# cgmb/euler

Hardware: AMD Instinct MI355X
Metric: cells*steps/sec of sim_step() (frames incl. the PCG pressure projection) + pressure-solve HBM GB/s vs roofline (higher is better)
Workload: dtype f64

## Files before the change

euler_amd/csrc/k_pcg.h:

```cpp
#pragma once

#include "euler_dev.h"
#include "k_mg.h"

#define COMM_CALL(expr) do { if ((expr) != 0) { eu_set_error("communicator callback failed: %s", #expr); return EULER_ECOMM; } } while (0)
#define LOC(ptr) ((ptr) + S->e_lo)
enum { SW_FACTOR = 0, SW_FORWARD = 1, SW_BACKWARD = 2 };

int eu_launch_build_system(euler_sim* S, float dt);
int eu_launch_velocity_update(euler_sim* S, float dt, int finish);
int eu_launch_band_ranges(euler_sim* S);
int eu_launch_sweep(euler_sim* S, int op, int cls, int force, int fin_qq = -1);
int eu_launch_factor_tile(euler_sim* S, int force);
int eu_launch_precond_tile(euler_sim* S, int rupd, int sweeps, int fin_dot, int force, double alpha, bool r_only = false, int zform = -1);
int eu_launch_search_apply(euler_sim* S, int it);
int eu_launch_finish_p(euler_sim* S);
int eu_launch_dot(euler_sim* S, const double* a, const double* b, int fin_op, int force);
int eu_comm_exchange(euler_sim* S, double* send_lo, double* send_hi, double* recv_lo, double* recv_hi, int count, double* small, int nsmall);
int eu_comm_finish(euler_sim* S, int fin_op, int is_max, int force);
int eu_comm_halo_two(euler_sim* S, double* a, double* b);
bool tile_recompute(const euler_sim* S);
int p_steps(const euler_sim* S);

enum { FIN_SIGMA_INIT = 0, FIN_ALPHA, FIN_RNORM, FIN_BETA, FIN_STORE_ONLY, FIN_TO_COMM };
#define FIN_VIA_P2P 0x100

static inline bool tile_fused(const euler_sim* S) { return eu_is_tile(S) && S->cfg.sweep_mode != EULER_SWEEP_SIMPLE; }
static inline bool ghost_mode(const euler_sim* S) { return S->has_comm && !S->p2p_on && tile_fused(S); }
enum { XR_ZSEND_LO = 0, XR_ZSEND_HI, XR_ZRECV_LO, XR_ZRECV_HI, XR_GS_LO0, XR_GS_LO1, XR_GS_HI0, XR_GS_HI1 };
static inline double* xrow(const euler_sim* S, int k) { return S->xrows + (size_t)k * S->xrow_len; }
static inline int sa_run(const euler_sim* S) {
  if (S->opt[EULER_OPT_SA_RUN] != 8 && !S->has_comm && !eu_is_two_level(S)) return (int)S->opt[EULER_OPT_SA_RUN];
  return 8;
}
static inline bool tile_z_recompute(const euler_sim* S) {
  return tile_recompute(S) && tile_fused(S) && !eu_is_two_level(S) && S->tile_w == 16 && !S->has_comm && !S->slab_on && S->band_lo == 0 &&
         S->opt[EULER_OPT_TILE_STORE_Z] == 0 && S->chunk_list && S->tile_table;
}
static inline int fin_or_comm(const euler_sim* S, int fin_op) {
  return S->has_comm ? (S->p2p_on ? (fin_op | FIN_VIA_P2P) : (int)FIN_TO_COMM) : fin_op;
}

#ifdef __HIPCC__
#define RED_THREADS 1024
typedef double sw_d2 __attribute__((ext_vector_type(2)));

__device__ __forceinline__ bool pcg_idle(const PcgScalars* sc) { return sc->done || !sc->nonzero; }

#define DPP_WAVE_SHL1 0x130
#define DPP_WAVE_SHR1 0x138

template <int CTRL>
__device__ __forceinline__ double wave_shift_inject(double v, double edge) {
  const int lo = __builtin_amdgcn_update_dpp(__double2loint(edge), __double2loint(v), CTRL, 0xf, 0xf, false);
  const int hi = __builtin_amdgcn_update_dpp(__double2hiint(edge), __double2hiint(v), CTRL, 0xf, 0xf, false);
  return __hiloint2double(hi, lo);
}


__device__ __forceinline__ void pcg_scalar_step(PcgScalars* sc, int op, double v) {
  switch (op) {
    case FIN_SIGMA_INIT: sc->sigma = v; break;
    case FIN_ALPHA: sc->zs = v; sc->alpha_prev = sc->alpha; sc->alpha = sc->sigma / v; sc->alpha_hist[sc->iters & 7] = sc->alpha; sc->iters += 1; break;
    case FIN_RNORM: sc->rnorm = v; if (v <= sc->tol) sc->done = 1; break;
    case FIN_BETA: sc->sigma_new = v; sc->beta = v / sc->sigma; sc->sigma = v; break;
    case FIN_TO_COMM: sc->comm_val = v; if (sc->comm_slot) *sc->comm_slot = v; break;
    default: sc->sigma_new = v; break;
// ... 113 lines not shown
  double* pre;
  const double* in;
  double* out;
  unsigned long long* granules;
  int gran_stride;
  const unsigned long long* xg_in;
  unsigned long long* xg_out;
  const int4* ranges;
  int band_lo, nb_local;
  int couple;
  unsigned int* ticket;
  unsigned int ticket_base;
  unsigned int epoch;
  const PcgScalars* sc;
  int force;
  int* error;
  unsigned long long* timeline;
  int tile_w;
  int fin_qq;
  double* qq_partial;
  unsigned int* qq_counter;
  PcgScalars* sc_w;
};

struct TileArgs {
  SkewGeom g;
  const uint8_t* mask;
  double* pre;
  double* r;
  const double* as;
  double* z;
  int band_lo, nb_local;
  int rupd;
  int sweeps;
  int fin_dot;
  int via;
  double* part_max; double* part_dot;
  unsigned int* counter;
  const unsigned int* list;
  const double* table;
  PcgScalars* sc;
  int force;
  double alpha_arg;
  double* pair_slot;
  double *zsend_lo, *zsend_hi;
  int edge_lo, edge_hi;
  int reverse;
  double* cpart;
  int cshift;
  int cmode, cnx, cny;
  const double *gs_lo, *gs_hi;
  int zform;
  double *zhalo, *zrows;
};

__device__ __forceinline__ double factor_step(double aa, double own, double nbv) {
  const double cl = -1.0 * own, cb = -1.0 * nbv;
  double e = aa - cl * cl - cb * cb;
  if (e < 0.25 * aa) e = (aa != 0.0) ? aa : 1.0;
  return 1.0 / sqrt(e);
}

template <int CTRL>
__device__ __forceinline__ double dpp_move(double v) {
  const int lo = __builtin_amdgcn_update_dpp(0, __double2loint(v), CTRL, 0xf, 0xf, true);
  const int hi = __builtin_amdgcn_update_dpp(0, __double2hiint(v), CTRL, 0xf, 0xf, true);
  return __hiloint2double(hi, lo);
}
__device__ __forceinline__ double group_sum(double v) {
  v = v + dpp_move<0xB1>(v);
  v = v + dpp_move<0x4E>(v);
  if (MG_LG == 8) v = v + dpp_move<0x141>(v);
  return v;
}
#endif
```

euler_amd/csrc/k_pcg.hip:

```cpp
#include "k_pcg.h"

#include <cmath>
#include <vector>

template <bool IS_MAX>
__global__ __launch_bounds__(RED_THREADS) void k_reduce_final(const double* __restrict__ partial, int n, PcgScalars* sc,
                                                              int op, int force) {
  if (!force && pcg_idle(sc)) return;
  double v = 0.0;
  for (int i = threadIdx.x; i < n; i += RED_THREADS) {
    const double w = partial[i];
    if (IS_MAX) v = w > v ? w : v; else v += w;
  }
  v = IS_MAX ? block_max(v) : block_sum(v);
  if (threadIdx.x == 0) pcg_scalar_step(sc, op, v);
}

template <bool EDGES>
__global__ __launch_bounds__(RED_THREADS) void k_dot_partial(const double* __restrict__ a, const double* __restrict__ b,
                                                             const uint8_t* __restrict__ mask, size_t S,
                                                             double* __restrict__ partial, PcgScalars* sc, int force,
                                                             unsigned int* counter, int fin_op, int TS, int nb_local, int edges) {
  if (!force && pcg_idle(sc)) return;
  const size_t chunk = (((S + gridDim.x - 1) / gridDim.x) + 1) & ~(size_t)1;
// ... 471 lines not shown
    hipLaunchKernelGGL(k_nonzero_to_comm, dim3(1), dim3(1), 0, S->stream, S->sc);
    COMM_CALL(S->comm.allreduce(S->comm.ctx, &S->sc->comm_val, 1, 1));
    hipLaunchKernelGGL(k_nonzero_from_comm, dim3(1), dim3(1), 0, S->stream, S->sc);
  }
  return EULER_OK;
}

static int project_resident(euler_sim* S, float dt, Solve& v) {
  const bool res_skip = S->res_skip_once != 0;
  S->res_skip_once = 0;
  if (!res_skip && eu_resident_eligible(S)) {
    const unsigned int cap_chunks = 4u * (unsigned int)eu_resident_capacity(S, S->cfg.pcg_precision == EULER_PCG_F32);
    unsigned int guess = S->res_last_chunks;
    if (!S->res_have_last) {
      HIPCHK(hipMemcpyAsync(S->sc_host, S->sc, sizeof(PcgScalars), hipMemcpyDeviceToHost, S->stream));
      HIPCHK(hipStreamSynchronize(S->stream));
      guess = S->sc_host->n_chunks;
    }
    if (guess + guess / 16 + 8 <= cap_chunks || S->cfg.pcg_precision == EULER_PCG_F32) {
      v.solved = true;
      S->prof_iter = -2;
      if (int rc = eu_launch_resident(S, cap_chunks)) return rc;
      HIPCHK(hipMemcpyAsync(S->sc_host, S->sc, sizeof(PcgScalars), hipMemcpyDeviceToHost, S->stream));
      HIPCHK(hipStreamSynchronize(S->stream));
      S->res_last_chunks = S->sc_host->n_chunks; S->res_have_last = 1;
      const int err = *S->res_err;
      if (err == 0) {
        if (S->sc_host->nonzero) { S->res_solves += 1; S->pcg_fields_resident = 1; }
        return eu_launch_velocity_update(S, dt, 0);
      }
      *S->res_err = 0;
      if (S->cfg.pcg_precision == EULER_PCG_F32 && err == 2) { eu_set_error("EULER_PCG_F32: the solve's active chunks do not fit the resident solver"); return EULER_EHIP; }
      if (err != 2) { S->res_fallbacks += 1; S->res_disabled = 1; }
      S->solve_seq -= 1;
      S->lean_ok = 0;
      S->res_skip_once = 1;
      *S->sc_host = v.prev;
      return eu_launch_project(S, dt);
    }
  }
  return EULER_OK;
}

static int project_first_direction(euler_sim* S, Solve& v) {
  int rc;
  const bool tile = tile_fused(S), two_level = tile && eu_is_two_level(S);
  if (two_level && S->has_comm && !(eu_is_mg(S) && ghost_mode(S) && S->slab_on)) {
    eu_set_error("coarse-correction preconditioners with several ranks: EULER_PRECOND_IC0_TILE_MG on row slabs without mailboxes only");
    return EULER_EINVAL;
  }
  if (two_level && (rc = eu_launch_coarse_setup(S))) return rc;
  if (two_level && (rc = eu_launch_coarse_consistent(S))) return rc;
  v.zr = tile && tile_z_begin(S);
  if (tile) {
    if ((rc = eu_launch_factor_tile(S, 0))) return rc;
    if ((rc = eu_launch_precond_tile(S, 0, 1, FIN_SIGMA_INIT, 0, 0.0))) return rc;
  } else {
  if (S->cfg.precond != EULER_PRECOND_JACOBI && (rc = eu_launch_sweep(S, SW_FACTOR, KC_PRECON_FACTOR, 0))) return rc;
  if ((rc = launch_precondition(S, 0, FIN_SIGMA_INIT))) return rc;
  }
  if ((rc = ring_begin(S))) return rc;
  if (first_direction_folded(S)) {
    const PcgScalars& ps = v.prev;
    if (ps.nonzero && !(std::isfinite(ps.alpha) && std::isfinite(ps.beta) && std::isfinite(ps.rnorm) && std::isfinite(ps.sigma) && std::isfinite(ps.zs)))
      for (int k = 0; k < S->s_ring_n; ++k) HIPCHK(hipMemsetAsync(S->s_ring[k] + S->skew_off, 0, S->Sw * sizeof(double), S->stream));
  }
  else if (two_level) { if ((rc = eu_launch_coarse_search_init(S))) return rc; }
  else
  LAUNCH(S, KC_UPDATE_SEARCH, k_update_search<true>, dim3(eu_blocks(S->e_cnt, 256 * 4, 4096)), dim3(256), LOC(S->s), LOC(S->z),
         LOC(S->cellmask), S->e_cnt, S->sc, 0, 0.0);
  if (S->has_comm && eu_p2p_has_neighbour_arrays(S)) {
    const int y0 = S->band_lo > 0 ? 64 * S->band_lo : -1, y1 = S->band_hi < S->geom.nbands ? 64 * S->band_hi - 1 : -1;
    LAUNCH(S, KC_UPDATE_SEARCH, k_publish_edge_rows, dim3((S->X + 255) / 256, 2), dim3(256), S->s, S->geom, y0, y1, S->sc);
  }
  if (S->s_ring_n == 2) HIPCHK(hipMemsetAsync(LOC(S->s2), 0, S->e_cnt * sizeof(double), S->stream));
  S->s_stale = 1;
  return EULER_OK;
}

static int project_iterate(euler_sim* S, Solve& v) {
  int rc;
  HIPCHK(hipMemcpyAsync(S->sc_host, S->sc, sizeof(PcgScalars), hipMemcpyDeviceToHost, S->stream));
  HIPCHK(hipStreamSynchronize(S->stream));
  const int poll = S->cfg.pcg_poll_interval > 0 ? S->cfg.pcg_poll_interval : 8;
  const int max_it = S->cfg.max_iterations;
  const bool tile = tile_fused(S), fold0 = first_direction_folded(S);
  int it = 0, chunk = 0;
  bool stop = !S->sc_host->nonzero;
  S->s_none = stop ? 1 : 0;
  while (it < max_it && !stop) {
    int chunk_end = it + poll;
    if (!v.drain_poll && v.pred_iters > 0 && it < v.pred_iters + poll && chunk_end > v.pred_iters - 2) {
      const int lo = v.pred_iters - 2 < chunk_end ? v.pred_iters - 2 : chunk_end;
      chunk_end = lo > it + 2 ? lo : it + 2;
    }
    if (chunk_end > max_it) chunk_end = max_it;
    for (; it < chunk_end; ++it) {
      S->prof_iter = it;
      const bool fused = it > 0 || fold0;
      if (it == 0 && fold0) { S->s = S->s_ring[S->s_ring_n - 1]; S->s2 = S->s_ring[0]; }
      if ((rc = fused ? eu_launch_search_apply(S, it) : launch_apply_a_and_alpha(S, 0))) return rc;
      if (tile) {
        S->prof_iter = it;
        const int nx = it + 1, steps = S->s_ring_n;
        const bool next_odd = !(nx >= steps && nx % steps == 0);
        const int zform = v.zr && it + 1 < max_it ? (it + 2 < max_it && next_odd ? 1 : 0) : -1;
        if ((rc = eu_launch_precond_tile(S, 1, it + 1 < max_it, FIN_BETA, 0, 0.0, false, zform))) return rc;
        S->z_halo_last = zform == 1;
        v.zr_ran = v.zr_ran || zform == 1;
        continue;
      }
      S->tile_as_override = fused ? S->q : S->z;
      rc = eu_launch_precond_tile(S, 1, 0, -1, 0, 0.0, true);
      S->tile_as_override = nullptr;
      if (rc) return rc;
      if (it + 1 < max_it) {
        S->prof_iter = it + 1;
        if ((rc = launch_precondition(S, 0, FIN_BETA))) return rc;
      }
    }
    if (it < max_it && v.drain_poll) {
      HIPCHK(hipMemcpyAsync(S->sc_host, S->sc, sizeof(PcgScalars), hipMemcpyDeviceToHost, S->stream));
      HIPCHK(hipStreamSynchronize(S->stream));
      stop = S->sc_host->done != 0;
    } else
    if (it < max_it) {
      const int slot = chunk & 1;
      if (chunk > 0) {
        HIPCHK(hipEventSynchronize(S->poll_event[slot ^ 1]));
        stop = S->poll_host[slot ^ 1].done != 0;
      }
      HIPCHK(hipMemcpyAsync(&S->poll_host[slot], S->sc, sizeof(PcgScalars), hipMemcpyDeviceToHost, S->stream));
      HIPCHK(hipEventRecord(S->poll_event[slot], S->stream));
      ++chunk;
    }
  }
  return EULER_OK;
}

static int project_finish(euler_sim* S, float dt, const Solve& v) {
  int rc;
  S->prof_iter = -2;
  S->z_halo_last = 0;
  if (v.zr_ran && (rc = eu_launch_precond_tile(S, 0, 1, -1, 0, 0.0, false, 2))) return rc;
  const bool finish_in_update = !S->has_comm && !S->slab_on && S->opt[EULER_OPT_VELOCITY_TWO_PASS] == 0;
  if (!finish_in_update) { if ((rc = eu_launch_finish_p(S))) return rc; }
  if (S->s_ring_n > 2) { S->s = S->s_base[0]; S->s2 = S->s_base[1]; }
  if (S->has_comm && S->slab_on) {
    const int X = S->X, nbk = (X + 255) / 256;
    double *send_lo = S->halo_buf, *send_hi = S->halo_buf + X, *recv_lo = S->halo_buf + 2 * X, *recv_hi = S->halo_buf + 3 * X;
    if (S->band_lo > 0) hipLaunchKernelGGL(k_pack_row, dim3(nbk), dim3(256), 0, S->stream, S->p, send_lo, S->geom, S->band_lo, 0);
    COMM_CALL(S->bulk.halo(S->bulk.ctx, send_lo, send_hi, recv_lo, recv_hi, X));
    if (S->band_hi < S->geom.nbands) hipLaunchKernelGGL(k_unpack_row, dim3(nbk), dim3(256), 0, S->stream, S->p, recv_hi, S->geom, S->band_hi, 0);
  } else if (S->has_comm) {
    const int n = S->comm.nranks, nb = S->geom.nbands;
    std::vector<int64_t> off(n), cnt(n);
    for (int k = 0; k < n; ++k) {
      const int64_t lo = (int64_t)nb * k / n, hi = (int64_t)nb * (k + 1) / n;
      off[k] = lo * S->geom.TS * 64 * 8;
// ... 65 lines not shown
```

euler_amd/csrc/k_search.hip:

```cpp
#include "k_pcg.h"

#include <type_traits>

#define SA_THREADS 256
struct SaPair { sw_d2 z, so; double ez0, es0, ez1, es1; };

__device__ __forceinline__ double pick3(int t, int tb1, int tb2, double v0, double v1, double v2) {
  double v = v0;
  v = t >= tb1 ? v1 : v;
  v = t >= tb2 ? v2 : v;
  return v;
}
template <int SLAB, int PMODE, int SA_RUN, int COARSE = 0, bool STORE = true, bool ZR = false>
__global__ __launch_bounds__(SA_THREADS, (COARSE == 2 && PMODE == 1 && SLAB == 0) ? 4 : 1) void k_search_apply(const double* __restrict__ s_old, const double* __restrict__ z,
                                                             double* __restrict__ s_new, double* __restrict__ out,
                                                             const uint8_t* __restrict__ mask, SkewGeom g,
                                                             double* __restrict__ partial, PcgScalars* sc, int force,
                                                             unsigned int* counter, int fin_op, SlabNeighbours nbr,
                                                             double* __restrict__ p, double* s_new_base, double* s_old_base,
                                                             const unsigned int* __restrict__ chunk_list,
                                                             CoarseRef cref, SaHist hist, ZrArgs zr) {
  static_assert(PMODE == 1 || PMODE == 2 || PMODE == 4 || PMODE == 8, "PMODE: p is left alone (1) or takes the N fmadds that are due (the ring's length)");
  static_assert(!ZR || (SLAB == 0 && SA_RUN == 8 && COARSE == 0), "ZR: one GPU, runs of one tile, no coarse part");
  __shared__ double s_cy[COARSE == 2 ? SA_THREADS / 64 : 1][COARSE == 2 ? MG_NI + 1 : 1][64];
  __shared__ double s_ce[COARSE == 2 ? SA_THREADS / 64 : 1][COARSE == 2 ? MG_NI + 1 : 1][64];
  if (!force && pcg_idle(sc)) return;
  __shared__ sw_d2 s_ztab[ZR ? 8 : 1][64];
  if (ZR) {
    for (int k = threadIdx.x; k < 8 * 64; k += SA_THREADS) (&s_ztab[0][0])[k] = reinterpret_cast<const sw_d2*>(zr.table)[k];
    __syncthreads();
  }
  const double beta = sc->beta;
  (void)s_new_base; (void)s_old_base;
  constexpr int NPA = PMODE >= 2 ? PMODE : 2;
  double al[NPA] = {};
  if (PMODE >= 2) {
    const int k = sc->iters;
#pragma unroll
    for (int j = 0; j < NPA; ++j) al[j] = sc->alpha_hist[(k - NPA + j) & 7];
  }
  const int lane = threadIdx.x & 63;
  const int TS = g.TS, npairs = TS / 2;
  const int nb_local = (int)(g.S / ((size_t)TS * 64));
  const int cpb = (npairs + SA_RUN - 1) / SA_RUN, total = nb_local * cpb;
  const int n_waves = gridDim.x * (SA_THREADS / 64);
  const bool edge_lane = lane == 0 || lane == 63;
  double t = 0.0;
  const bool listed = chunk_list != nullptr;
  const int ntb16 = g.T / 16;
  const int todo = listed ? (int)sc->n_chunks : total;
  typedef std::integral_constant<bool, true> yes_t;
  typedef std::integral_constant<bool, false> no_t;
  for (int i = blockIdx.x * (SA_THREADS / 64) + (threadIdx.x >> 6); i < todo; i += n_waves) {
    int c = i, per = cpb;
    bool interior = false;
    if (listed) { const unsigned int ent = chunk_list[i]; interior = (ent & EU_CHUNK_INTERIOR) != 0; c = (int)(ent & ~EU_CHUNK_INTERIOR); per = ntb16; }
    const int lb = c / per, P0 = (c % per) * SA_RUN, P1 = ZR ? P0 + SA_RUN : (P0 + SA_RUN < npairs ? P0 + SA_RUN : npairs);
    const size_t bbase = (size_t)lb * TS * 64 + 2 * lane;
    auto run = [&](auto full_tag) {
      constexpr bool FULL = decltype(full_tag)::value;
      unsigned int mm[SA_RUN];
      unsigned int any = 0;
#pragma unroll
      for (int j = 0; j < SA_RUN; ++j) {
        if (FULL) mm[j] = CM_INTERIOR | (CM_INTERIOR << 8);
        else mm[j] = P0 + j < P1 ? (unsigned int)*reinterpret_cast<const unsigned short*>(mask + bbase + (size_t)(P0 + j) * 128) : 0u;
        any |= mm[j];
      }
      if (!FULL && !listed && !__ballot(((any | (any >> 8)) & CM_FLUID) != 0)) return;
      sw_d2 zz[ZR ? SA_RUN : 1];
      if (ZR) {
        sw_d2 rr[SA_RUN], pp[SA_RUN];
#pragma unroll
        for (int j = 0; j < SA_RUN; ++j) {
          rr[j] = *reinterpret_cast<const sw_d2*>(zr.r + bbase + (size_t)(P0 + j) * 128);
          pp[j] = FULL ? s_ztab[j][lane] : *reinterpret_cast<const sw_d2*>(zr.pre + bbase + (size_t)(P0 + j) * 128);
        }
        double none = 0.0;
        tile_solve<2 * SA_RUN, false>(mm, rr, pp, zz, none);
      }
      const int ztile = P0 / SA_RUN;
      const bool up_remote = SLAB == 1 && nbr.z_up && lb + 1 == nb_local, dn_remote = SLAB == 1 && nbr.z_dn && lb == 0;
      const double* ez = lane == 0 ? (dn_remote ? nbr.z_dn : z) : (up_remote ? nbr.z_up : z);
      const double* es = lane == 0 ? (dn_remote ? nbr.s_dn : s_old) : (up_remote ? nbr.s_up : s_old);
      const bool remote = lane == 0 ? dn_remote : up_remote;
      const long long e0_base = lane == 0 ? ((long long)(lb - 1) * TS + 62) * 64 + 127 : ((long long)(lb + 1) * TS - 64) * 64 + 1;
      const long long e1_base = lane == 0 ? ((long long)(lb - 1) * TS + 64) * 64 + 126 : ((long long)(lb + 1) * TS - 62) * 64;
      const unsigned int vbit = lane == 0 ? CM_DOWN : CM_UP;
      const bool ghost = SLAB == 2 && (lane == 0 ? (nbr.zrow_dn != nullptr && lb == 0) : (nbr.zrow_up != nullptr && lb + 1 == nb_local));
      const double* gz = lane == 0 ? nbr.zrow_dn : nbr.zrow_up;
      const double* gs = lane == 0 ? nbr.srow_dn : nbr.srow_up;
      double* gsn = lane == 0 ? nbr.snew_dn : nbr.snew_up;
      const int gcol = lane == 0 ? 0 : -63;
      const double* zrow = ZR ? zr.rows + (long long)(lane == 0 ? 2 * lb - 1 : 2 * lb + 2) * zr.X : nullptr;
      double cy0 = 0.0, cy1 = 0.0, cy2 = 0.0, ce0 = 0.0, ce1 = 0.0, ce2 = 0.0;
      double (*cyv)[64] = s_cy[COARSE == 2 ? threadIdx.x >> 6 : 0];
      double (*cev)[64] = s_ce[COARSE == 2 ? threadIdx.x >> 6 : 0];
      int ctb1 = 0x7fffffff, ctb2 = 0x7fffffff, cJb = 0;
      (void)cJb;
      if (COARSE == 2) {
        cJb = (2 * (P0 - 1) - lane - MG_G0 / 2) >> MG_LOG;
        ctb1 = MG_G0 * (cJb + 1) + lane + MG_G0 / 2;
        const int row = (cref.band0 + lb) * 64 + lane;
        const int hi_ = cref.nx - 1;
        int i0, i1;
        double fy;
        mg_cell_w(row, cref.ny, i0, i1, fy);
        const double* y0 = cref.y + (size_t)i0 * cref.nx;
        const double* y1 = cref.y + (size_t)i1 * cref.nx;
#pragma unroll
        for (int q = 0; q <= MG_NI; ++q) { const int c = cJb + q < 0 ? 0 : (cJb + q < hi_ ? cJb + q : hi_); cyv[q][lane] = mg_rows(y0[c], y1[c], fy); }
#pragma unroll
        for (int q = 0; q <= MG_NI; ++q) cev[q][lane] = 0.0;
        if (edge_lane) {
          const int re = row + (lane == 0 ? -1 : 1);
          if (re >= 0 && re < MG_G0 * cref.ny) {
            mg_cell_w(re, cref.ny, i0, i1, fy);
            y0 = cref.y + (size_t)i0 * cref.nx; y1 = cref.y + (size_t)i1 * cref.nx;
#pragma unroll
            for (int q = 0; q <= MG_NI; ++q) { const int c = cJb + q < 0 ? 0 : (cJb + q < hi_ ? cJb + q : hi_); cev[q][lane] = mg_rows(y0[c], y1[c], fy); }
          }
        }
// ... 40 lines not shown
            if (ZR) { d.ez0 = zrow[2 * P + gcol]; d.es0 = s_old[k]; }
            else if (SLAB == 2 && ghost) { d.ez0 = gz[2 * P + gcol]; d.es0 = gs[2 * P + gcol]; }
            else if (SLAB == 1 && remote) { d.ez0 = ld_system(ez + k); d.es0 = ld_system(es + k); } else { d.ez0 = ez[k]; d.es0 = es[k]; }
          }
          if (((m >> 8) & CM_FLUID) && ((m >> 8) & vbit)) {
            const long long k = e1_base + (long long)P * 128;
            if (ZR) { d.ez1 = zrow[2 * P + 1 + gcol]; d.es1 = s_old[k]; }
            else if (SLAB == 2 && ghost) { d.ez1 = gz[2 * P + 1 + gcol]; d.es1 = gs[2 * P + 1 + gcol]; }
            else if (SLAB == 1 && remote) { d.ez1 = ld_system(ez + k); d.es1 = ld_system(es + k); } else { d.ez1 = ez[k]; d.es1 = es[k]; }
          }
          if (COARSE == 1) {
            d.ez0 = d.ez0 + pick3(2 * P, ctb1, ctb2, ce0, ce1, ce2);
            d.ez1 = d.ez1 + pick3(2 * P + 1, ctb1, ctb2, ce0, ce1, ce2);
          }
          if (COARSE == 2) {
            d.ez0 = d.ez0 + p0y(2 * P, cev);
            d.ez1 = d.ez1 + p0y(2 * P + 1, cev);
          }
        }
        if (COARSE == 1) {
          d.z.x = d.z.x + pick3(2 * P, ctb1, ctb2, cy0, cy1, cy2);
          d.z.y = d.z.y + pick3(2 * P + 1, ctb1, ctb2, cy0, cy1, cy2);
        }
        if (COARSE == 2) {
          d.z.x = d.z.x + p0y(2 * P, cyv);
          d.z.y = d.z.y + p0y(2 * P + 1, cyv);
        }
      };
      auto sprime = [&](const SaPair& d) __attribute__((always_inline)) { return sw_d2{d.z.x + beta * d.so.x, d.z.y + beta * d.so.y}; };
      SaPair A, B, Cn;
      load_pair(P0 - 1, A, 0u);
      load_pair(P0, B, mm[0]);
      load_pair(P0 + 1, Cn, SA_RUN > 1 ? mm[1] : 0u);
      double prev_y = sprime(A).y;
      sw_d2 cur = sprime(B);
#pragma unroll
      for (int j = 0; j < SA_RUN; ++j) {
        const int P = P0 + j;
        if (P < P1) {
          SaPair D;
          load_pair(P + 2 <= P1 ? P + 2 : -1, D, j + 2 < SA_RUN ? mm[j + 2] : 0u);
          const unsigned int m0 = mm[j] & 0xff, m1 = mm[j] >> 8;
          const sw_d2 nxt = sprime(Cn);
          const double e0 = B.ez0 + beta * B.es0, e1 = B.ez1 + beta * B.es1;
          if (SLAB == 2 && ghost && edge_lane) {
            if ((mm[j] & CM_FLUID) && (mm[j] & vbit)) gsn[2 * P + gcol] = e0;
            if (((mm[j] >> 8) & CM_FLUID) && ((mm[j] >> 8) & vbit)) gsn[2 * P + 1 + gcol] = e1;
          }
          const double dn0 = wave_shift_inject<DPP_WAVE_SHR1>(prev_y, e0), up0 = wave_shift_inject<DPP_WAVE_SHL1>(cur.y, e0);
          const double dn1 = wave_shift_inject<DPP_WAVE_SHR1>(cur.x, e1), up1 = wave_shift_inject<DPP_WAVE_SHL1>(nxt.x, e1);
          if ((m0 | m1) & CM_FLUID) {
            const size_t i = bbase + (size_t)P * 128;
            sw_d2 cc = B.so, o = {0.0, 0.0};
            if (PMODE >= 2) {
              sw_d2 pv = *reinterpret_cast<const sw_d2*>(p + i);
              constexpr int NP = PMODE >= 2 ? PMODE : 2;
              sw_d2 sv[NP];
              sv[0] = *reinterpret_cast<const sw_d2*>(s_new + i);
#pragma unroll
              for (int j = 1; j < NP - 1; ++j) sv[j] = *reinterpret_cast<const sw_d2*>(hist.s[j - 1] + i);
              sv[NP - 1] = B.so;
#pragma unroll
              for (int j = 0; j < NP; ++j) {
                if (m0 & CM_FLUID) pv.x = pv.x + sv[j].x * al[j];
                if (m1 & CM_FLUID) pv.y = pv.y + sv[j].y * al[j];
              }
              *reinterpret_cast<sw_d2*>(p + i) = pv;
            }
            if (m0 & CM_FLUID) cc.x = cur.x;
            if (m1 & CM_FLUID) cc.y = cur.y;
            if (m0 & CM_FLUID) {
              double v = (double)(int)(m0 >> CM_DIAG_SHIFT) * cc.x;
              v = v - ((m0 & CM_RIGHT) ? cc.y : 0.0);
              v = v - ((m0 & CM_UP) ? up0 : 0.0);
              v = v - ((m0 & CM_LEFT) ? prev_y : 0.0);
              v = v - ((m0 & CM_DOWN) ? dn0 : 0.0);
              o.x = v;
              t += v * cc.x;
            }
            if (m1 & CM_FLUID) {
              double v = (double)(int)(m1 >> CM_DIAG_SHIFT) * cc.y;
              v = v - ((m1 & CM_RIGHT) ? nxt.x : 0.0);
              v = v - ((m1 & CM_UP) ? up1 : 0.0);
              v = v - ((m1 & CM_LEFT) ? cc.x : 0.0);
              v = v - ((m1 & CM_DOWN) ? dn1 : 0.0);
              o.y = v;
              t += v * cc.y;
            }
            if ((m0 & m1) & CM_FLUID) *reinterpret_cast<sw_d2*>(s_new + i) = cc;
            else if (m0 & CM_FLUID) s_new[i] = cc.x;
            else s_new[i + 1] = cc.y;
            if (STORE) {
              if ((m0 & m1) & CM_FLUID) *reinterpret_cast<sw_d2*>(out + i) = o;
              else if (m0 & CM_FLUID) out[i] = o.x;
              else out[i + 1] = o.y;
            }
            if (SLAB == 1 && slab_edge_row(i, lane, TS, nb_local, (nbr.z_dn ? 1 : 0) | (nbr.z_up ? 2 : 0))) {
              if (m0 & CM_FLUID) st_system(s_new + i, cc.x);
              if (m1 & CM_FLUID) st_system(s_new + i + 1, cc.y);
            }
          }
          prev_y = cur.y; cur = nxt;
          B = Cn; Cn = D;
        }
      }
    };
    if (SA_RUN == 8 && interior) run(yes_t()); else run(no_t());
// ... 6 lines not shown
static inline unsigned sa_blocks(const euler_sim* S, int run) {
  return eu_blocks((size_t)(S->band_hi - S->band_lo) * ((S->geom.TS / 2 + run - 1) / run), SA_THREADS / 64, 2048);
}
struct SaCall { SkewGeom gl; int fin; SlabNeighbours nbr; CoarseRef cref; SaHist hist; ZrArgs zr; };
template <int SLAB, int PMODE, int RUN, int COARSE, bool STORE, bool ZR = false>
static void sa_launch(euler_sim* S, const SaCall& c) {
  LAUNCH(S, KC_APPLY_A, (k_search_apply<SLAB, PMODE, RUN, COARSE, STORE, ZR>), dim3(sa_blocks(S, RUN)), dim3(SA_THREADS), LOC(S->s), LOC(S->z), LOC(S->s2),
         LOC(S->q), LOC(S->cellmask), c.gl, S->partial, S->sc, 0, S->red_counter, c.fin, c.nbr, LOC(S->p), S->s2, S->s, RUN == 8 ? S->chunk_list : (const unsigned int*)nullptr, c.cref, c.hist, c.zr);
}
template <int SLAB, int COARSE, int PMODE>
static void sa_pick_run(euler_sim* S, const SaCall& c, int run, bool store) {
  if constexpr (COARSE == 0 && SLAB != 2 && PMODE <= 2) {
    if constexpr (SLAB == 0) { if (run == 16) return sa_launch<SLAB, PMODE, 16, COARSE, true>(S, c); }
    if (run != 8) return sa_launch<SLAB, PMODE, 32, COARSE, true>(S, c);
  }
  if (store) sa_launch<SLAB, PMODE, 8, COARSE, true>(S, c); else sa_launch<SLAB, PMODE, 8, COARSE, false>(S, c);
}
template <int SLAB, int COARSE>
static void sa_pick(euler_sim* S, const SaCall& c, int pmode, int run, bool store) {
  if constexpr (SLAB != 1) {
    if (pmode == 8) return sa_pick_run<SLAB, COARSE, 8>(S, c, run, store);
    if (pmode == 4) return sa_pick_run<SLAB, COARSE, 4>(S, c, run, store);
  }
  if (pmode == 2) sa_pick_run<SLAB, COARSE, 2>(S, c, run, store); else sa_pick_run<SLAB, COARSE, 1>(S, c, run, store);
}
int eu_launch_search_apply(euler_sim* S, int it) {
  const bool seq = S->cfg.dot_mode == EULER_DOT_SEQUENTIAL && !S->has_comm;
  SlabNeighbours nbr = {nullptr, nullptr, nullptr, nullptr, S->band_hi - S->band_lo, nullptr, nullptr, nullptr, nullptr, nullptr, nullptr};
  const bool direct = S->has_comm && eu_p2p_has_neighbour_arrays(S);
  const bool ghost = ghost_mode(S);
  if (ghost) {
    const int c = S->gs_cur;
    if (S->band_lo > 0) { nbr.zrow_dn = xrow(S, XR_ZRECV_LO); nbr.srow_dn = xrow(S, XR_GS_LO0 + c); nbr.snew_dn = xrow(S, XR_GS_LO0 + (c ^ 1)); }
    if (S->band_hi < S->geom.nbands) { nbr.zrow_up = xrow(S, XR_ZRECV_HI); nbr.srow_up = xrow(S, XR_GS_HI0 + c); nbr.snew_up = xrow(S, XR_GS_HI0 + (c ^ 1)); }
    S->gs_cur = c ^ 1;
  } else if (direct) {
    eu_p2p_neighbour_arrays(S, &nbr.z_dn, &nbr.s_dn, &nbr.z_up, &nbr.s_up);
    if (nbr.z_dn) { nbr.z_dn += S->e_lo; nbr.s_dn += S->e_lo; }
    if (nbr.z_up) { nbr.z_up += S->e_lo; nbr.s_up += S->e_lo; }
  } else if (S->has_comm) {
    if (int rc = eu_comm_halo_two(S, S->z, S->s)) return rc;
  }
  const int steps = S->s_ring_n;
  const int pmode = (it >= steps && it % steps == 0) ? steps : 1;
  const bool mg = eu_is_mg(S);
  SaCall c = {S->geom, S->has_comm ? fin_or_comm(S, FIN_ALPHA) : (seq ? -1 : (int)FIN_ALPHA), nbr,
              {mg ? S->mg_x : S->cc_y, mg ? 0 : S->coarse_shift, mg ? S->mg_nx[0] : S->coarse_nx, mg ? S->mg_ny[0] : S->coarse_ny, S->band_lo},
              {{nullptr, nullptr, nullptr, nullptr, nullptr, nullptr}}, {S->r, S->precon, S->tile_table, S->zhalo, S->zrows, S->X}};
  c.gl.S = S->e_cnt;
  for (int j = 1; j + 1 < steps; ++j) c.hist.s[j - 1] = LOC(S->s_ring[j]);
  const int run = sa_run(S);
  const bool store = !tile_recompute(S);
  const bool coarse = eu_is_two_level(S) && tile_fused(S);
  if (S->z_halo_last) sa_launch<0, 1, 8, 0, false, true>(S, c);
  else if (coarse && ghost) sa_pick<2, 2>(S, c, pmode, run, store);
  else if (coarse && mg) sa_pick<0, 2>(S, c, pmode, run, store);
  else if (coarse) sa_pick<0, 1>(S, c, pmode, run, store);
  else if (ghost) sa_pick<2, 0>(S, c, pmode, run, store);
  else if (direct) sa_pick<1, 0>(S, c, pmode, run, store);
  else sa_pick<0, 0>(S, c, pmode, run, store);
  S->s = S->s_ring[it % steps]; S->s2 = S->s_ring[(it + 1) % steps];
  S->s_launched = it + 1;
  if (seq) eu_launch_dot(S, S->q, S->s, FIN_ALPHA, 0);
  return S->has_comm ? eu_comm_finish(S, FIN_ALPHA, 0, 0) : EULER_OK;
}
```

euler_amd/csrc/k_tile.hip:

```cpp
#include "k_pcg.h"

#include <type_traits>

#define PT_THREADS 256
__device__ __forceinline__ void tile_block_reduce(double& mx, double& sm) {
  __shared__ double s_mx[PT_THREADS / 64], s_sm[PT_THREADS / 64];
  mx = eu_wave_max(mx);
  sm = eu_wave_sum(sm);
  __syncthreads();
  if ((threadIdx.x & 63) == 0) { s_mx[threadIdx.x >> 6] = mx; s_sm[threadIdx.x >> 6] = sm; }
  __syncthreads();
  if (threadIdx.x == 0) {
    mx = s_mx[0]; sm = s_sm[0];
    for (int k = 1; k < PT_THREADS / 64; ++k) { mx = s_mx[k] > mx ? s_mx[k] : mx; sm += s_sm[k]; }
  }
}

__global__ __launch_bounds__(64) void k_tile_table(double* __restrict__ tab) {
  const int lane = threadIdx.x & 63;
  double own = 0.0, out = 0.0;
  sw_d2 pp[8];
#pragma unroll
  for (int j = 0; j < 16; ++j) {
    const double nbv = wave_shift_inject<DPP_WAVE_SHR1>(out, 0.0);
// ... 192 lines not shown
          if ((lane & 3) == 0) { sp[quad * 2 * MG_NSLOT + q] = p0; sp[quad * 2 * MG_NSLOT + MG_NSLOT + q] = p1; }
        }
        __builtin_amdgcn_fence(__ATOMIC_RELEASE, "wavefront");
        __builtin_amdgcn_wave_barrier();
        {
          double* cp = a.cpart + ((size_t)(tile / ntb) * MG_NGRP * ntb + (size_t)k) * (2 * MG_NSLOT);
#pragma unroll
          for (int u = 0; u < (MG_PART + 63) / 64; ++u) {
            const int e = lane + 64 * u;
            if (e < MG_PART) {
              const int g = e / (2 * MG_NSLOT), w = e % (2 * MG_NSLOT);
              const double va = g > 0 ? sp[(2 * g - 1) * 2 * MG_NSLOT + w] : 0.0, vb = g < 8 ? sp[(2 * g) * 2 * MG_NSLOT + w] : 0.0;
              cp[((size_t)g * ntb) * (2 * MG_NSLOT) + w] = va + vb;
            }
          }
        }
        __builtin_amdgcn_fence(__ATOMIC_ACQUIRE, "wavefront");
        __builtin_amdgcn_wave_barrier();
      } else if (W == 16 && CMODE == 1) {
        const int xl = k * W - 63, J0 = (xl > 0 ? xl : 0) >> a.cshift;
        double c0 = 0.0, c1 = 0.0, c2 = 0.0;
#pragma unroll
        for (int j = 0; j < W; ++j) {
          const int cm = (int)((mm[j >> 1] >> ((j & 1) * 8)) & 0xff);
          const double rv = (cm & CM_FLUID) ? ((j & 1) ? rr[j >> 1].y : rr[j >> 1].x) : 0.0;
          const int x = k * W + j - lane;
          const int b = ((x > 0 ? x : 0) >> a.cshift) - J0;
          c0 += b == 0 ? rv : 0.0; c1 += b == 1 ? rv : 0.0; c2 += b == 2 ? rv : 0.0;
        }
        c0 = eu_wave_sum(c0); c1 = eu_wave_sum(c1); c2 = eu_wave_sum(c2);
        if (lane == 0) { double* cp = a.cpart + (size_t)tile * 3; cp[0] = c0; cp[1] = c1; cp[2] = c2; }
      }
      if (RECOMP && a.rupd) {
        asm volatile("" ::: "memory");
#pragma unroll
        for (int P = 0; P < W / 2; ++P) pp[P] = FULL ? s_tab[P < TABP ? P : 0][lane] : *reinterpret_cast<const sw_d2*>(a.pre + base + P * 128);
      }
      tile_solve<W, true>(mm, rr, pp, qq, dsum);
      if (W == 16 && a.zform == 1) {
        double* h = a.zhalo + ((size_t)band * ntb + k) * 128;
        h[lane] = qq[0].x;
        h[64 + lane] = qq[W / 2 - 1].y;
        if (lane == 0 || lane == 63) {
          double* row = a.zrows + ((size_t)band * 2 + (lane == 63 ? 1 : 0)) * a.g.X;
#pragma unroll
          for (int j = 0; j < W; ++j) {
            const int x = k * W + j - lane;
            if (x >= 0 && x < a.g.X) row[x] = (j & 1) ? qq[j >> 1].y : qq[j >> 1].x;
          }
        }
      } else {
#pragma unroll
        for (int P = 0; P < W / 2; ++P) *reinterpret_cast<sw_d2*>(a.z + base + P * 128) = qq[P];
      }
      if (band == a.edge_lo || band == a.edge_hi) {
        const bool lo = band == a.edge_lo && lane == 0, hi = band == a.edge_hi && lane == 63;
#pragma unroll
        for (int j = 0; j < W; ++j) {
          const double zv = (j & 1) ? qq[j >> 1].y : qq[j >> 1].x;
          const int x_lo = k * W + j, x_hi = k * W + j - 63;
          if (lo && x_lo < a.g.X) a.zsend_lo[x_lo] = zv;
          if (hi && x_hi >= 0 && x_hi < a.g.X) a.zsend_hi[x_hi] = zv;
        }
      }
    };
    if (W == 16 && interior) run(yes_t()); else run(no_t());
  }
  tile_block_reduce(mx, dsum);
  __shared__ int am_last;
  if (threadIdx.x == 0) {
    __hip_atomic_store(reinterpret_cast<unsigned long long*>(&a.part_max[blockIdx.x]), (unsigned long long)__double_as_longlong(mx), __ATOMIC_RELAXED, __HIP_MEMORY_SCOPE_AGENT);
    __hip_atomic_store(reinterpret_cast<unsigned long long*>(&a.part_dot[blockIdx.x]), (unsigned long long)__double_as_longlong(dsum), __ATOMIC_RELAXED, __HIP_MEMORY_SCOPE_AGENT);
    asm volatile("s_waitcnt vmcnt(0)" ::: "memory");
    const unsigned int t = __hip_atomic_fetch_add(a.counter, 1u, __ATOMIC_RELAXED, __HIP_MEMORY_SCOPE_AGENT);
    am_last = t == gridDim.x - 1;
  }
  __syncthreads();
  if (!am_last) return;
  double vmax = 0.0, vsum = 0.0;
  for (unsigned int i = threadIdx.x; i < gridDim.x; i += PT_THREADS) {
    const double m = __longlong_as_double((long long)__hip_atomic_load(reinterpret_cast<unsigned long long*>(&a.part_max[i]), __ATOMIC_RELAXED, __HIP_MEMORY_SCOPE_AGENT));
    const double d = __longlong_as_double((long long)__hip_atomic_load(reinterpret_cast<unsigned long long*>(&a.part_dot[i]), __ATOMIC_RELAXED, __HIP_MEMORY_SCOPE_AGENT));
    vmax = m > vmax ? m : vmax; vsum += d;
  }
  tile_block_reduce(vmax, vsum);
  if (a.via == FIN_VIA_P2P) {
    if (a.rupd) vmax = p2p_allreduce_block<true>(a.sc, vmax);
    if (a.fin_dot >= 0) vsum = p2p_allreduce_block<false>(a.sc, vsum);
  }
  if (threadIdx.x == 0) {
    if (a.via == FIN_TO_COMM) { a.pair_slot[0] = vmax; a.pair_slot[1] = vsum; }
    else {
      if (a.rupd) pcg_scalar_step(a.sc, FIN_RNORM, vmax);
      if (a.fin_dot >= 0 && !(a.rupd && a.sc->done)) pcg_scalar_step(a.sc, a.fin_dot, vsum);
    }
    if (a.zform >= 0) a.sc->zfix = a.zform == 1 ? 1u : 0u;
    __hip_atomic_store(a.counter, 0u, __ATOMIC_RELAXED, __HIP_MEMORY_SCOPE_AGENT);
  }
}

__global__ void k_pair_fold(PcgScalars* sc, const double* __restrict__ pairs, int stride, int R, int rupd, int fin_dot, int force) {
  if (!force && pcg_idle(sc)) return;
  double vmax = 0.0, vsum = 0.0;
  for (int r = 0; r < R; ++r) { vmax = pairs[(size_t)stride * r] > vmax ? pairs[(size_t)stride * r] : vmax; vsum += pairs[(size_t)stride * r + 1]; }
  if (rupd) pcg_scalar_step(sc, FIN_RNORM, vmax);
  if (fin_dot >= 0 && !(rupd && sc->done)) pcg_scalar_step(sc, fin_dot, vsum);
}
static TileArgs make_tile_args(euler_sim* S, int force) {
  TileArgs a;
  a.g = S->geom; a.mask = S->cellmask; a.pre = S->precon; a.r = S->r; a.as = S->tile_as_override ? S->tile_as_override : S->q; a.z = S->z;
  a.band_lo = S->band_lo; a.nb_local = S->band_hi - S->band_lo;
  a.rupd = 0; a.sweeps = 1; a.fin_dot = -1;
  a.via = S->has_comm ? (S->p2p_on ? (int)FIN_VIA_P2P : (int)FIN_TO_COMM) : 0;
  a.part_max = S->partial; a.part_dot = S->partial2; a.counter = S->red_counter; a.sc = S->sc; a.force = force; a.alpha_arg = 0.0;
  a.pair_slot = S->pair_buf + 2 * (S->has_comm ? S->comm.rank : 0);
  a.list = !force ? S->chunk_list : nullptr;
  a.table = S->tile_table;
  a.zsend_lo = a.zsend_hi = nullptr; a.edge_lo = a.edge_hi = -1;
  a.reverse = S->opt[EULER_OPT_TILE_REVERSE] != 0;
  a.cpart = nullptr; a.cshift = 0; a.cmode = 0; a.cnx = a.cny = 0;
  a.gs_lo = a.gs_hi = nullptr;
  a.zform = -1; a.zhalo = S->zhalo; a.zrows = S->zrows;
  if (ghost_mode(S)) {
    if (S->band_lo > 0) { a.zsend_lo = xrow(S, XR_ZSEND_LO); a.edge_lo = S->band_lo; }
    if (S->band_hi < S->geom.nbands) { a.zsend_hi = xrow(S, XR_ZSEND_HI); a.edge_hi = S->band_hi - 1; }
  }
  return a;
}
static inline unsigned tile_blocks(const euler_sim* S, int w) {
  return eu_blocks((size_t)(S->band_hi - S->band_lo) * (S->geom.T / w), PT_THREADS / 64, 2048);
}
typedef void (*TileKernel)(TileArgs);
int eu_launch_factor_tile(euler_sim* S, int force) {
  const TileKernel k = S->tile_w == 8 ? k_factor_tile<8> : S->tile_w == 32 ? k_factor_tile<32> : k_factor_tile<16>;
  LAUNCH(S, KC_PRECON_FACTOR, k, dim3(tile_blocks(S, S->tile_w)), dim3(PT_THREADS), make_tile_args(S, force));
  return EULER_OK;
}
int eu_launch_precond_tile(euler_sim* S, int rupd, int sweeps, int fin_dot, int force, double alpha, bool r_only, int zform) {
  const bool seq = S->cfg.dot_mode == EULER_DOT_SEQUENTIAL && !S->has_comm;
  TileArgs a = make_tile_args(S, force);
  a.rupd = rupd; a.sweeps = sweeps; a.fin_dot = (seq || !sweeps) ? -1 : fin_dot; a.alpha_arg = alpha;
  a.zform = zform;
  const bool two_level = eu_is_two_level(S) && sweeps && !r_only && !force && a.list != nullptr;
  const int fin_real = a.fin_dot;
  if (two_level) {
    const bool mg = eu_is_mg(S);
    a.cpart = mg ? S->mg_part : S->cc_part; a.cshift = mg ? 0 : S->coarse_shift;
    a.cmode = mg ? 2 : 1; a.cnx = mg ? S->mg_nx[0] : 0; a.cny = mg ? S->mg_ny[0] : 0;
    if (a.fin_dot >= 0) a.fin_dot = FIN_STORE_ONLY;
  }
  double* xsmall = S->pair_buf;
  int nsmall = 2;
  bool split = false;
  if (two_level && a.via == FIN_TO_COMM) {
    split = eu_is_mg(S) && ghost_mode(S) && eu_mg_split(S);
    nsmall = eu_coarse_comm_slots(S);
    if (nsmall < 0) return EULER_ENOMEM;
    xsmall = S->mg_xbuf;
    a.pair_slot = xsmall + (size_t)S->comm.rank * nsmall;
    if (split) {
      if (a.zsend_lo) a.zsend_lo = eu_mg_split_msg(S, 0);
      if (a.zsend_hi) a.zsend_hi = eu_mg_split_msg(S, 1);
    }
  }
  const int w = r_only ? 16 : S->tile_w, cls = r_only ? KC_UPDATE_PR : zform == 2 ? KC_MISC : KC_PRECOND_TILE;
  const bool recomp = rupd && !force && tile_recompute(S) && (r_only ? S->tile_as_override == S->q : !S->tile_as_override);
  if (recomp) {
    a.as = S->s;
    if (ghost_mode(S)) {
      if (S->band_lo > 0) a.gs_lo = xrow(S, XR_GS_LO0 + S->gs_cur);
      if (S->band_hi < S->geom.nbands) a.gs_hi = xrow(S, XR_GS_HI0 + S->gs_cur);
    }
  }
  const TileKernel k = w == 8 ? k_precond_tile<8> : w == 32 ? k_precond_tile<32>
                     : a.cmode == 2 ? (recomp ? k_precond_tile<16, true, 2> : k_precond_tile<16, false, 2>)
                     : a.cmode == 1 ? (recomp ? k_precond_tile<16, true, 1> : k_precond_tile<16, false, 1>)
                     : (recomp ? k_precond_tile<16, true> : k_precond_tile<16>);
  LAUNCH(S, cls, k, dim3(tile_blocks(S, w)), dim3(PT_THREADS), a);
  if (two_level && a.via != FIN_TO_COMM) { int rc = eu_launch_coarse_solve(S, fin_real, force); if (rc) return rc; }
  if (seq && sweeps && fin_dot >= 0) eu_launch_dot(S, S->z, S->r, fin_dot, force);
  if (a.via == FIN_TO_COMM) {
    const int R = S->comm.nranks;
    const bool rows = ghost_mode(S) && !force;
    int rc = !two_level ? EULER_OK : split ? eu_mg_split_pre(S) : eu_launch_coarse_pre(S, force);
    if (rc) return rc;
    if (split) rc = eu_comm_exchange(S, eu_mg_split_msg(S, 0), eu_mg_split_msg(S, 1), eu_mg_split_msg(S, 2), eu_mg_split_msg(S, 3), eu_mg_split_count(S), xsmall, nsmall);
    else rc = eu_comm_exchange(S, xrow(S, XR_ZSEND_LO), xrow(S, XR_ZSEND_HI), xrow(S, XR_ZRECV_LO), xrow(S, XR_ZRECV_HI), rows ? S->X : 0, xsmall, nsmall);
    if (rc) return rc;
    hipLaunchKernelGGL(k_pair_fold, dim3(1), dim3(1), 0, S->stream, S->sc, xsmall, nsmall, R, rupd, a.fin_dot, force);
    if (split) {
      if ((rc = eu_mg_split_mid(S, fin_real, force, xrow(S, XR_ZRECV_LO), xrow(S, XR_ZRECV_HI)))) return rc;
      if ((rc = eu_comm_exchange(S, nullptr, nullptr, nullptr, nullptr, 0, eu_mg_split_gc(S), 1 + MG_NULL_MAX))) return rc;
      return eu_mg_split_fold(S, fin_real, force);
    }
    if (two_level) { rc = eu_launch_coarse_scatter(S); if (rc) return rc; rc = eu_launch_coarse_solve(S, fin_real, force); if (rc) return rc; }
// ... 4 lines not shown
```

Before: 194.7 million.

## Fuse initial search-direction write into tile precond and extend z-form to eight-step ring

The first preconditioner tile launch now also writes z into the first search-ring buffer, so the separate k_update_search launch that copied z into s is skipped on that path. The z-forming schedule is extended so that with an 8-deep search ring every iteration forms z. A new search-apply variant with PMODE 8 and the ZR path folds the p += sum(alpha*s) update ahead of the z work, instead of doing it in the later loop. This saves one kernel launch and a full-vector pass at solve start and merges work across stages. In exchange the tile kernel does extra stores and the search kernel has more register pressure.

Result: slower. 191.2 million (-1.8%).

```diff
diff --git a/euler_amd/csrc/k_pcg.h b/euler_amd/csrc/k_pcg.h
--- a/euler_amd/csrc/k_pcg.h
+++ b/euler_amd/csrc/k_pcg.h
@@ -12,7 +12,7 @@
 int eu_launch_band_ranges(euler_sim* S);
 int eu_launch_sweep(euler_sim* S, int op, int cls, int force, int fin_qq = -1);
 int eu_launch_factor_tile(euler_sim* S, int force);
-int eu_launch_precond_tile(euler_sim* S, int rupd, int sweeps, int fin_dot, int force, double alpha, bool r_only = false, int zform = -1);
+int eu_launch_precond_tile(euler_sim* S, int rupd, int sweeps, int fin_dot, int force, double alpha, bool r_only = false, int zform = -1, double* s0 = nullptr);
 int eu_launch_search_apply(euler_sim* S, int it);
 int eu_launch_finish_p(euler_sim* S);
 int eu_launch_dot(euler_sim* S, const double* a, const double* b, int fin_op, int force);
@@ -232,6 +232,7 @@
   const double *gs_lo, *gs_hi;
   int zform;
   double *zhalo, *zrows;
+  double* s0;
 };
 
 __device__ __forceinline__ double factor_step(double aa, double own, double nbv) {
diff --git a/euler_amd/csrc/k_pcg.hip b/euler_amd/csrc/k_pcg.hip
--- a/euler_amd/csrc/k_pcg.hip
+++ b/euler_amd/csrc/k_pcg.hip
@@ -547,21 +547,22 @@
   if (two_level && (rc = eu_launch_coarse_setup(S))) return rc;
   if (two_level && (rc = eu_launch_coarse_consistent(S))) return rc;
   v.zr = tile && tile_z_begin(S);
+  if ((rc = ring_begin(S))) return rc;
+  const bool s0_in_tile = v.zr && !two_level && !first_direction_folded(S);
   if (tile) {
     if ((rc = eu_launch_factor_tile(S, 0))) return rc;
-    if ((rc = eu_launch_precond_tile(S, 0, 1, FIN_SIGMA_INIT, 0, 0.0))) return rc;
+    if ((rc = eu_launch_precond_tile(S, 0, 1, FIN_SIGMA_INIT, 0, 0.0, false, -1, s0_in_tile ? S->s_ring[0] : nullptr))) return rc;
   } else {
   if (S->cfg.precond != EULER_PRECOND_JACOBI && (rc = eu_launch_sweep(S, SW_FACTOR, KC_PRECON_FACTOR, 0))) return rc;
   if ((rc = launch_precondition(S, 0, FIN_SIGMA_INIT))) return rc;
   }
-  if ((rc = ring_begin(S))) return rc;
   if (first_direction_folded(S)) {
     const PcgScalars& ps = v.prev;
     if (ps.nonzero && !(std::isfinite(ps.alpha) && std::isfinite(ps.beta) && std::isfinite(ps.rnorm) && std::isfinite(ps.sigma) && std::isfinite(ps.zs)))
       for (int k = 0; k < S->s_ring_n; ++k) HIPCHK(hipMemsetAsync(S->s_ring[k] + S->skew_off, 0, S->Sw * sizeof(double), S->stream));
   }
   else if (two_level) { if ((rc = eu_launch_coarse_search_init(S))) return rc; }
-  else
+  else if (!s0_in_tile)
   LAUNCH(S, KC_UPDATE_SEARCH, k_update_search<true>, dim3(eu_blocks(S->e_cnt, 256 * 4, 4096)), dim3(256), LOC(S->s), LOC(S->z),
          LOC(S->cellmask), S->e_cnt, S->sc, 0, 0.0);
   if (S->has_comm && eu_p2p_has_neighbour_arrays(S)) {
@@ -598,8 +599,8 @@
       if (tile) {
         S->prof_iter = it;
         const int nx = it + 1, steps = S->s_ring_n;
-        const bool next_odd = !(nx >= steps && nx % steps == 0);
-        const int zform = v.zr && it + 1 < max_it ? (it + 2 < max_it && next_odd ? 1 : 0) : -1;
+        const bool next_forms_z = !(nx >= steps && nx % steps == 0) || steps == 8;
+        const int zform = v.zr && it + 1 < max_it ? (it + 2 < max_it && next_forms_z ? 1 : 0) : -1;
         if ((rc = eu_launch_precond_tile(S, 1, it + 1 < max_it, FIN_BETA, 0, 0.0, false, zform))) return rc;
         S->z_halo_last = zform == 1;
         v.zr_ran = v.zr_ran || zform == 1;
diff --git a/euler_amd/csrc/k_search.hip b/euler_amd/csrc/k_search.hip
--- a/euler_amd/csrc/k_search.hip
+++ b/euler_amd/csrc/k_search.hip
@@ -68,6 +68,27 @@
         any |= mm[j];
       }
       if (!FULL && !listed && !__ballot(((any | (any >> 8)) & CM_FLUID) != 0)) return;
+      if (ZR && PMODE >= 2) {
+        constexpr int NP = PMODE >= 2 ? PMODE : 2;
+#pragma unroll
+        for (int j = 0; j < SA_RUN; ++j) {
+          const unsigned int m0 = mm[j] & 0xff, m1 = mm[j] >> 8;
+          const size_t i = bbase + (size_t)(P0 + j) * 128;
+          sw_d2 pv = *reinterpret_cast<const sw_d2*>(p + i);
+          sw_d2 sv[NP];
+          sv[0] = *reinterpret_cast<const sw_d2*>(s_new + i);
+#pragma unroll
+          for (int q = 1; q < NP - 1; ++q) sv[q] = *reinterpret_cast<const sw_d2*>(hist.s[q - 1] + i);
+          sv[NP - 1] = *reinterpret_cast<const sw_d2*>(s_old + i);
+#pragma unroll
+          for (int q = 0; q < NP; ++q) {
+            if (m0 & CM_FLUID) pv.x = pv.x + sv[q].x * al[q];
+            if (m1 & CM_FLUID) pv.y = pv.y + sv[q].y * al[q];
+          }
+          *reinterpret_cast<sw_d2*>(p + i) = pv;
+        }
+        asm volatile("" ::: "memory");
+      }
       sw_d2 zz[ZR ? SA_RUN : 1];
       if (ZR) {
         sw_d2 rr[SA_RUN], pp[SA_RUN];
@@ -214,7 +235,7 @@
           if ((m0 | m1) & CM_FLUID) {
             const size_t i = bbase + (size_t)P * 128;
             sw_d2 cc = B.so, o = {0.0, 0.0};
-            if (PMODE >= 2) {
+            if (PMODE >= 2 && !ZR) {
               sw_d2 pv = *reinterpret_cast<const sw_d2*>(p + i);
               constexpr int NP = PMODE >= 2 ? PMODE : 2;
               sw_d2 sv[NP];
@@ -327,7 +348,8 @@
   const int run = sa_run(S);
   const bool store = !tile_recompute(S);
   const bool coarse = eu_is_two_level(S) && tile_fused(S);
-  if (S->z_halo_last) sa_launch<0, 1, 8, 0, false, true>(S, c);
+  if (S->z_halo_last && pmode == 8) sa_launch<0, 8, 8, 0, false, true>(S, c);
+  else if (S->z_halo_last) sa_launch<0, 1, 8, 0, false, true>(S, c);
   else if (coarse && ghost) sa_pick<2, 2>(S, c, pmode, run, store);
   else if (coarse && mg) sa_pick<0, 2>(S, c, pmode, run, store);
   else if (coarse) sa_pick<0, 1>(S, c, pmode, run, store);
diff --git a/euler_amd/csrc/k_tile.hip b/euler_amd/csrc/k_tile.hip
--- a/euler_amd/csrc/k_tile.hip
+++ b/euler_amd/csrc/k_tile.hip
@@ -268,6 +268,10 @@
       } else {
 #pragma unroll
         for (int P = 0; P < W / 2; ++P) *reinterpret_cast<sw_d2*>(a.z + base + P * 128) = qq[P];
+        if (!RECOMP && W == 16 && a.s0) {
+#pragma unroll
+          for (int P = 0; P < W / 2; ++P) *reinterpret_cast<sw_d2*>(a.s0 + base + P * 128) = qq[P];
+        }
       }
       if (band == a.edge_lo || band == a.edge_hi) {
         const bool lo = band == a.edge_lo && lane == 0, hi = band == a.edge_hi && lane == 63;
@@ -336,7 +340,7 @@
   a.reverse = S->opt[EULER_OPT_TILE_REVERSE] != 0;
   a.cpart = nullptr; a.cshift = 0; a.cmode = 0; a.cnx = a.cny = 0;
   a.gs_lo = a.gs_hi = nullptr;
-  a.zform = -1; a.zhalo = S->zhalo; a.zrows = S->zrows;
+  a.zform = -1; a.zhalo = S->zhalo; a.zrows = S->zrows; a.s0 = nullptr;
   if (ghost_mode(S)) {
     if (S->band_lo > 0) { a.zsend_lo = xrow(S, XR_ZSEND_LO); a.edge_lo = S->band_lo; }
     if (S->band_hi < S->geom.nbands) { a.zsend_hi = xrow(S, XR_ZSEND_HI); a.edge_hi = S->band_hi - 1; }
@@ -352,11 +356,11 @@
   LAUNCH(S, KC_PRECON_FACTOR, k, dim3(tile_blocks(S, S->tile_w)), dim3(PT_THREADS), make_tile_args(S, force));
   return EULER_OK;
 }
-int eu_launch_precond_tile(euler_sim* S, int rupd, int sweeps, int fin_dot, int force, double alpha, bool r_only, int zform) {
+int eu_launch_precond_tile(euler_sim* S, int rupd, int sweeps, int fin_dot, int force, double alpha, bool r_only, int zform, double* s0) {
   const bool seq = S->cfg.dot_mode == EULER_DOT_SEQUENTIAL && !S->has_comm;
   TileArgs a = make_tile_args(S, force);
   a.rupd = rupd; a.sweeps = sweeps; a.fin_dot = (seq || !sweeps) ? -1 : fin_dot; a.alpha_arg = alpha;
-  a.zform = zform;
+  a.zform = zform; a.s0 = s0;
   const bool two_level = eu_is_two_level(S) && sweeps && !r_only && !force && a.list != nullptr;
   const int fin_real = a.fin_dot;
   if (two_level) {
```
